# rrwick/Deepbinner

Hardware: AMD Instinct MI355X
Metric: reads classified/sec (1024-sample windows, batch 256) (higher is better)
Workload: dtype f32

## Files before the change

deepbinner_amd/csrc/dbh_api.hip:

```cpp
#include <hip/hip_runtime.h>

#include <algorithm>
#include <cmath>
#include <cstdio>
#include <cstdlib>
#include <cstring>
#include <new>
#include <string>
#include <thread>
#include <utility>
#include <mutex>
#include <vector>

#include "../../include/deepbinner_hip.h"
#include "dbh_general.h"
#define DBH_FORWARD_NS dbh
#define DBH_TIMELINE 0
#include "dbh_forward.hip"
#undef DBH_FORWARD_NS
#undef DBH_TIMELINE
#define DBH_FORWARD_NS dbh_timeline
#define DBH_TIMELINE 1
#include "dbh_forward.hip"
#undef DBH_FORWARD_NS
#undef DBH_TIMELINE

namespace {

thread_local std::string g_last_error;

int hip_fail(hipError_t e, const char* what) {
    g_last_error = std::string(what) + ": " + hipGetErrorString(e);
    return e == hipErrorOutOfMemory ? DBH_ERR_OUT_OF_MEMORY : DBH_ERR_HIP;
}

#define DBH_HIP(call)                                         \
    do {                                                      \
        hipError_t e_ = (call);                               \
        if (e_ != hipSuccess) return hip_fail(e_, #call);     \
    } while (0)

struct CanonConv { int k, cin, cout; };
void canon_convs(int n_classes, CanonConv out[dbh::kNumConvs]) {
    for (int i = 0; i < dbh::kNumConvs; ++i) {
        out[i].k = dbh::kConv[i].taps;
        out[i].cin = dbh::kConv[i].cin;
        out[i].cout = (i == dbh::kNumConvs - 1) ? n_classes : dbh::kConv[i].cout_pad;
    }
}

int64_t canon_param_count(int n_classes) {
    CanonConv cc[dbh::kNumConvs];
    canon_convs(n_classes, cc);
    int64_t n = 0;
    for (int i = 0; i < dbh::kNumConvs; ++i) n += (int64_t)cc[i].k * cc[i].cin * cc[i].cout + cc[i].cout;
    for (int i = 0; i < dbh::kNumBn; ++i) n += 4 * dbh::kBnChannels[i];
    return n;
}

void pack_weights(const float* w, int n_classes, std::vector<float>& packed) {
    using namespace dbh;
    packed.assign(kPackedFloats, 0.f);
    CanonConv cc[kNumConvs];
    canon_convs(n_classes, cc);
    const float* bn_first = w;
    for (int i = 0; i < kNumConvs; ++i) bn_first += (size_t)cc[i].k * cc[i].cin * cc[i].cout + cc[i].cout;
    std::vector<double> fold_scale(48, 1.0), fold_shift(48, 0.0);
    {
        const float* q = bn_first + 4 * kBnChannels[0];
        const float *gamma = q, *beta = q + 48, *mean = q + 96, *var = q + 144;
        for (int c = 0; c < 48; ++c) {
            fold_scale[c] = (double)gamma[c] / std::sqrt((double)var[c] + 1e-3);
            fold_shift[c] = (double)beta[c] - (double)mean[c] * fold_scale[c];
        }
    }
    static_assert(kBnChannels[1] == 48 && kConv[4].cin == 48 && kConv[4].taps == 1, "");
    const float* p = w;
    for (int i = 0; i < kNumConvs; ++i) {
        const int k = cc[i].k, cin = cc[i].cin, cout = cc[i].cout;
        const float* kernel = p;
        const float* bias = p + (size_t)k * cin * cout;
        p = bias + cout;
        float* dst = packed.data() + weight_offset(i);
        if (i == 0) {
            for (int tap = 0; tap < 3; ++tap)
                for (int c = 0; c < cout; ++c) dst[tap * 48 + c] = kernel[(tap * cin) * cout + c];
        } else if (kConv[i].wino) {
            const int sp_n = cin / 8, nt = kConv[i].cout_pad / 16;
            const int n_xi = kConv[i].wino == 4 ? 6 : 4;
            static const double G23[4][3] = {{1, 0, 0}, {.5, .5, .5}, {.5, -.5, .5}, {0, 0, 1}};
            static const double G43[6][3] = {{1. / 4, 0, 0},
                                             {-1. / 6, -1. / 6, -1. / 6},
                                             {-1. / 6, 1. / 6, -1. / 6},
                                             {1. / 24, 1. / 12, 1. / 6},
                                             {1. / 24, -1. / 12, 1. / 6},
                                             {0, 0, 1}};
            for (int xi = 0; xi < n_xi; ++xi) {
                const double* G = kConv[i].wino == 4 ? G43[xi] : G23[xi];
                for (int sp = 0; sp < sp_n; ++sp)
                    for (int t = 0; t < nt; ++t)
                        for (int lane = 0; lane < 64; ++lane)
                            for (int e = 0; e < 2; ++e) {
                                const int ci = frag_cin(i, sp, lane >> 4, e);
                                const int co = 16 * t + (lane & 15);
                                double v = 0.0;
                                if (co < cout)
                                    for (int tap = 0; tap < 3; ++tap)
                                        v += G[tap] * (double)kernel[((size_t)tap * cin + ci) * cout + co];
                                const size_t idx =
                                    kConv[i].wino == 4
                                        ? (((((size_t)t * sp_n + sp) * 3 + (xi >> 1)) * 64 + lane) * 2 + (xi & 1)) * 2 + e
                                        : wino2_by_tile(i)
// ... 143 lines not shown

int launch_forward(dbh_model* m, const float* x_dev, int64_t n, float* probs_dev,
                   int debug_stage, float* debug_dev, hipStream_t stream,
                   const FusedInput& in = FusedInput()) {
    if (m->kind != DBH_MODEL_KIND_PERSISTENT) return DBH_ERR_UNSUPPORTED;
    if (n == 0) return DBH_OK;
    const int64_t kChunk = (int64_t)(1 << 20) * in.steps;
    for (int64_t off = 0; off < n; off += kChunk) {
        const int64_t cnt = (n - off < kChunk) ? (n - off) : kChunk;
        hipEvent_t ev_stop = nullptr;
        if (m->timing > 0 && (debug_stage < 0 || debug_stage >= 100)) {
            const int64_t pos = m->launch_counter++ % m->timing;
            if (pos == 0) {
                if (m->events_used == m->events.size()) {
                    hipEvent_t a, b;
                    DBH_HIP(hipEventCreate(&a));
                    DBH_HIP(hipEventCreate(&b));
                    m->events.emplace_back(a, b);
                }
                DBH_HIP(hipEventRecord(m->events[m->events_used].first, stream));
                m->open_stop = m->events[m->events_used].second;
                m->open_windows = 0;
            }
            if (m->open_stop && pos < m->timing_span) {
                m->open_windows += cnt;
                if (pos == m->timing_span - 1) {
                    ev_stop = m->open_stop;
                    m->open_stop = nullptr;
                }
            }
        }
        const bool one_per_group = debug_stage >= 0 && debug_stage != 301;
        const int64_t groups = (cnt + dbh::kGroup - 1) / dbh::kGroup;
        const unsigned grid = (unsigned)(one_per_group || groups < m->cus ? groups : m->cus);
        void** tail = in.tail;
        size_t* tail_bytes = in.tail_bytes;
        if (!tail) {
            size_t k = 0;
            while (k < m->tails.size() && m->tails[k].stream != stream) ++k;
            if (k == m->tails.size()) m->tails.push_back(dbh_model::Tail{stream, nullptr, 0});
            tail = &m->tails[k].ptr;
            tail_bytes = &m->tails[k].bytes;
        }
        {
            void* before = *tail;
            const int st = ensure(tail, tail_bytes, 256 + (size_t)grid * dbh::kWgScratchFloats * sizeof(float));
            if (st != DBH_OK) return st;
            if (*tail != before) DBH_HIP(hipMemsetAsync(*tail, 0, 256, stream));
        }
        dbh::ForwardArgs a;
        a.packed = m->d_packed;
        a.x = x_dev ? x_dev + off * dbh::kWindow : nullptr;
        a.probs = probs_dev ? probs_dev + off * m->n_classes : nullptr;
        a.debug_out = debug_dev ? debug_dev + off * dbh::kStageFloats[debug_stage < 0 || debug_stage > 7 ? 0 : debug_stage]
                                : nullptr;
        a.samples = in.samples;
        a.offsets = in.offsets ? (const long long*)(in.offsets + off / in.steps) : nullptr;
        a.calls = in.calls ? (int*)(in.calls + off / in.steps) : nullptr;
        a.tail_scratch = (float*)((char*)*tail + 256);
        a.win_counter = (debug_stage < 0 && m->windows_by_counter) ? (int*)*tail : nullptr;
        a.clock_out = nullptr;
        if (m->clock_probe && debug_stage < 0) {
            const int st = ensure(&m->d_clock, &m->clock_bytes,
                                  (size_t)grid * (4 + dbh::kPhaseMarks * dbh::kPhaseGroups) * sizeof(int64_t));
            if (st != DBH_OK) return st;
            a.clock_out = (long long*)m->d_clock;
            m->clock_grid = grid;
        }
        a.score_diff = in.score_diff;
        a.read0 = (long long)(in.read0 + off / in.steps);
        a.len_hint = (long long)in.len_hint;
        a.hint_cap = (long long)in.hint_cap;
        a.n_windows = (long long)cnt;
        a.n_classes = m->n_classes;
        a.debug_stage = debug_stage;
        a.steps = in.steps;
        a.side = in.side;
        a.phases = m->phase_probe ? 1 : 0;
        a.chunk4_min_left = m->chunk4_rounds * (int)grid;
        a.chunk2_min_left = m->chunk2_rounds * (int)grid;
        if (debug_stage == 300)
            hipLaunchKernelGGL(dbh_timeline::dbh_forward_kernel, dim3(grid), dim3(dbh::kThreads),
                               0, stream, reinterpret_cast<dbh_timeline::ForwardArgs&>(a));
        else
            hipLaunchKernelGGL(dbh::dbh_forward_kernel, dim3(grid), dim3(dbh::kThreads), 0, stream,
                               a);
        DBH_HIP(hipGetLastError());
        if (ev_stop) {
            DBH_HIP(hipEventRecord(ev_stop, stream));
            ++m->events_used;
            m->timed_windows += m->open_windows;
            m->timed_launches += m->timing_span;
        }
    }
    return DBH_OK;
}

inline int steps_for(int scan_size) { return scan_size / (dbh::kWindow / 2); }

inline int model_steps(const dbh_model* m, int scan_size) {
    const int half = m->input_size / 2;
    const int steps = scan_size / half;
    return (steps > 0 && steps * half == scan_size) ? steps : 0;
}

inline size_t align256(size_t bytes) { return (bytes + 255) & ~(size_t)255; }

size_t general_workspace(const dbh_model* m, int64_t n_reads, int steps) {
    const int64_t windows = n_reads * steps;
    return align256((size_t)windows * m->n_classes * sizeof(float)) +
           dbh_gen::activation_bytes(m->gen, windows);
}

int general_predict(dbh_model* m, const float* x_dev, int64_t n, float* probs_dev,
                    hipStream_t stream) {
    if (n == 0) return DBH_OK;
    size_t k = 0;
    while (k < m->gen_scratch.size() && m->gen_scratch[k].stream != stream) ++k;
    if (k == m->gen_scratch.size()) m->gen_scratch.push_back(dbh_model::Tail{stream, nullptr, 0});
    dbh_model::Tail& sc = m->gen_scratch[k];
    const int st = ensure(&sc.ptr, &sc.bytes, dbh_gen::activation_bytes(m->gen, n));
    if (st != DBH_OK) return st;
    DBH_HIP(dbh_gen::forward(m->gen, x_dev, nullptr, nullptr, 1, 0, n, probs_dev, sc.ptr, stream));
    return DBH_OK;
}

}

extern "C" {

const char* dbh_version(void) { return "deepbinner_hip 0.1 (gfx950)"; }

const char* dbh_status_string(int status) {
    switch (status) {
        case DBH_OK: return "ok";
        case DBH_ERR_INVALID_ARGUMENT: return "invalid argument";
        case DBH_ERR_NO_DEVICE: return "no HIP device available";
        case DBH_ERR_HIP: return "HIP runtime error";
        case DBH_ERR_BAD_WEIGHTS: return "weight blob does not match the Deepbinner architecture";
        case DBH_ERR_UNSUPPORTED: return "unsupported model geometry";
        case DBH_ERR_OUT_OF_MEMORY: return "out of device memory";
        case DBH_ERR_COMM: return "multi-device exchange failed";
        default: return "unknown status";
    }
}

const char* dbh_last_error(void) { return g_last_error.c_str(); }

int dbh_device_count(int* count) {
    if (!count) return DBH_ERR_INVALID_ARGUMENT;
    int n = 0;
    static const bool once = [] {
        const char* spin = std::getenv("DEEPBINNER_SPIN_WAIT");
        if (!(spin && spin[0] == '1')) {
            int devices = 0;
            if (hipGetDeviceCount(&devices) == hipSuccess)
                for (int d = 0; d < devices; ++d)
                    if (hipSetDevice(d) == hipSuccess)
                        (void)hipSetDeviceFlags(hipDeviceScheduleBlockingSync);
            if (devices > 0) (void)hipSetDevice(0);
            (void)hipGetLastError();
        }
        return true;
    }();
    (void)once;
    hipError_t e = hipGetDeviceCount(&n);
    if (e != hipSuccess) {
        *count = 0;
        hip_fail(e, "hipGetDeviceCount");
// ... 923 lines not shown
    int32_t* side_calls_host[2] = {start_calls_host, end_calls_host};
    for (int j = 0; j < 2; ++j)
        if (side_calls_host[j] && models[j])
            std::memcpy(side_calls_host[j],
                        h + in_small + ((const char*)d_side[j] - (const char*)d_status),
                        (size_t)n_reads * sizeof(int32_t));
    if (stream_status_host && n_streams) {
        const int32_t* sorted_status = (const int32_t*)(h + in_small);
        for (int64_t i = 0; i < n_streams; ++i)
            stream_status_host[order[(size_t)i]] = sorted_status[i];
    }
    if (stage_ms) {
        float ms = 0.f;
        for (int k = 0; k < 3; ++k) {
            stage_ms[k] = hipEventElapsedTime(&ms, ev[k], ev[k + 1]) == hipSuccess ? ms : -1.0;
        }
    }
    return done(DBH_OK);
}

void* dbh_host_alloc(size_t bytes, void* user) {
    (void)user;
    void* p = nullptr;
    if (hipHostMalloc(&p, bytes ? bytes : 1, hipHostMallocPortable) != hipSuccess) {
        (void)hipGetLastError();
        return nullptr;
    }
    return p;
}

void dbh_host_release(void* ptr, void* user) {
    (void)user;
    if (ptr) (void)hipHostFree(ptr);
}

int dbh_host_is_pinned(const void* ptr, size_t bytes, int* pinned) {
    if (!pinned) return DBH_ERR_INVALID_ARGUMENT;
    *pinned = is_pinned(ptr, bytes) ? 1 : 0;
    return DBH_OK;
}

int dbh_model_set_host_group(dbh_model* m, int64_t windows_per_group) {
    if (!m || windows_per_group < 0) return DBH_ERR_INVALID_ARGUMENT;
    if (m->kind != DBH_MODEL_KIND_PERSISTENT) return DBH_OK;
    m->host_group_windows = windows_per_group > 0 ? windows_per_group : dbh_model::kDefaultGroup;
    return DBH_OK;
}

int dbh_model_reserve_cus(dbh_model* m, int n_cus) {
    if (!m || n_cus < 0) return DBH_ERR_INVALID_ARGUMENT;
    if (m->kind != DBH_MODEL_KIND_PERSISTENT) return DBH_OK;
    m->cus = m->cus_total - n_cus > 1 ? m->cus_total - n_cus : 1;
    return DBH_OK;
}

int dbh_stage_floats(int stage, int64_t* floats_per_window) {
    if (!floats_per_window || stage < 0 || stage > 7) return DBH_ERR_INVALID_ARGUMENT;
    *floats_per_window = dbh::kStageFloats[stage];
    return DBH_OK;
}

int dbh_debug_forward(dbh_model* m, const float* x_host, int64_t n, int stage, float* out_host) {
    if (!m || n <= 0 || !x_host || !out_host || stage < 0 || stage > 7)
        return DBH_ERR_INVALID_ARGUMENT;
    if (m->kind != DBH_MODEL_KIND_PERSISTENT) return DBH_ERR_UNSUPPORTED;
    const size_t per = (size_t)dbh::kStageFloats[stage];
    int st = ensure(&m->d_in, &m->in_bytes, (size_t)n * dbh::kWindow * sizeof(float));
    if (st != DBH_OK) return st;
    st = ensure(&m->d_work, &m->work_bytes, (size_t)n * per * sizeof(float));
    if (st != DBH_OK) return st;
    DBH_HIP(hipMemcpyAsync(m->d_in, x_host, (size_t)n * dbh::kWindow * sizeof(float),
                           hipMemcpyHostToDevice, 0));
    DBH_HIP(hipMemsetAsync(m->d_work, 0, (size_t)n * per * sizeof(float), 0));
    st = launch_forward(m, (const float*)m->d_in, n, nullptr, stage, (float*)m->d_work, 0);
    if (st != DBH_OK) return st;
    DBH_HIP(hipMemcpyAsync(out_host, m->d_work, (size_t)n * per * sizeof(float),
                           hipMemcpyDeviceToHost, 0));
    DBH_HIP(hipStreamSynchronize(0));
    return DBH_OK;
}

int dbh_forward_kernel_info(int* threads_per_block, int* lds_bytes, int* vgprs) {
    hipFuncAttributes attr;
    DBH_HIP(hipFuncGetAttributes(&attr, (const void*)dbh::dbh_forward_kernel));
    if (threads_per_block) *threads_per_block = dbh::kThreads;
    if (lds_bytes) *lds_bytes = (int)attr.sharedSizeBytes;
    if (vgprs) *vgprs = attr.numRegs;
    return DBH_OK;
}

int dbh_forward_executed_mfmas(int n_classes, int64_t* mfmas_per_window,
                                int64_t* flop_per_window) {
    if (n_classes < 2 || n_classes > dbh::kMaxClasses) return DBH_ERR_INVALID_ARGUMENT;
    const int64_t n = dbh::forward_mfmas(n_classes);
    if (mfmas_per_window) *mfmas_per_window = n;
    if (flop_per_window) *flop_per_window = n * 2048;
    return DBH_OK;
}

int dbh_forward_truncated_dev(dbh_model* m, const float* x_dev, int64_t n, int last_stage,
                              dbh_stream stream) {
    if (!m || n <= 0 || !x_dev || last_stage < 0 || last_stage > 6) return DBH_ERR_INVALID_ARGUMENT;
    if (m->kind != DBH_MODEL_KIND_PERSISTENT) return DBH_ERR_UNSUPPORTED;
    return launch_forward(m, x_dev, n, nullptr, 100 + last_stage, nullptr, (hipStream_t)stream);
}

int dbh_forward_timeline(dbh_model* m, const float* x_host, int64_t n, int64_t* stamps_host) {
    if (!m || n <= 0 || !x_host || !stamps_host) return DBH_ERR_INVALID_ARGUMENT;
    if (m->kind != DBH_MODEL_KIND_PERSISTENT) return DBH_ERR_UNSUPPORTED;
    const size_t stamp_bytes = (size_t)n * dbh::kWaves * 64 * sizeof(int64_t);
    int st = ensure(&m->d_in, &m->in_bytes, (size_t)n * dbh::kWindow * sizeof(float));
    if (st != DBH_OK) return st;
    st = ensure(&m->d_work, &m->work_bytes, stamp_bytes);
    if (st != DBH_OK) return st;
    st = ensure(&m->d_out, &m->out_bytes, (size_t)n * m->n_classes * sizeof(float));
    if (st != DBH_OK) return st;
    DBH_HIP(hipMemcpyAsync(m->d_in, x_host, (size_t)n * dbh::kWindow * sizeof(float),
                           hipMemcpyHostToDevice, 0));
    DBH_HIP(hipMemsetAsync(m->d_work, 0, stamp_bytes, 0));
    {
        dbh_timeline::ForwardArgs a = {};
        a.packed = m->d_packed;
        a.x = (const float*)m->d_in;
        a.probs = (float*)m->d_out;
        a.debug_out = (float*)m->d_work;
        a.n_windows = (long long)n;
        a.n_classes = m->n_classes;
        a.debug_stage = 300;
        a.steps = 1;
        const unsigned grid = (unsigned)((n + dbh::kGroup - 1) / dbh::kGroup);
        st = ensure(&m->d_tail, &m->tail_bytes, (size_t)grid * dbh::kWgScratchFloats * sizeof(float));
        if (st != DBH_OK) return st;
        a.tail_scratch = (float*)m->d_tail;
        a.win_counter = nullptr;
        hipLaunchKernelGGL(dbh_timeline::dbh_forward_kernel, dim3(grid), dim3(dbh::kThreads), 0, 0, a);
    }
    DBH_HIP(hipGetLastError());
    DBH_HIP(hipMemcpyAsync(stamps_host, m->d_work, stamp_bytes, hipMemcpyDeviceToHost, 0));
    DBH_HIP(hipStreamSynchronize(0));
    return DBH_OK;
}

int dbh_forward_timeline_i16(dbh_model* m, const int16_t* samples_host, int64_t n,
                             int64_t* stamps_host) {
    if (!m || n <= 0 || !samples_host || !stamps_host) return DBH_ERR_INVALID_ARGUMENT;
    if (m->kind != DBH_MODEL_KIND_PERSISTENT) return DBH_ERR_UNSUPPORTED;
    const size_t stamp_bytes = (size_t)n * dbh::kWaves * 64 * sizeof(int64_t);
    const size_t sample_bytes = (size_t)n * dbh::kWindow * sizeof(int16_t);
    const size_t offset_bytes = (size_t)(n + 1) * sizeof(int64_t);
    int st = ensure(&m->d_in, &m->in_bytes, sample_bytes + offset_bytes + 16);
    if (st != DBH_OK) return st;
    st = ensure(&m->d_work, &m->work_bytes, stamp_bytes);
    if (st != DBH_OK) return st;
    st = ensure(&m->d_out, &m->out_bytes, (size_t)n * (m->n_classes + 1) * sizeof(float));
    if (st != DBH_OK) return st;
    std::vector<int64_t> offsets((size_t)n + 1);
    for (int64_t i = 0; i <= n; ++i) offsets[(size_t)i] = i * dbh::kWindow;
    char* d_offsets = (char*)m->d_in + ((sample_bytes + 7) & ~(size_t)7);
    DBH_HIP(hipMemcpyAsync(m->d_in, samples_host, sample_bytes, hipMemcpyHostToDevice, 0));
    DBH_HIP(hipMemcpyAsync(d_offsets, offsets.data(), offset_bytes, hipMemcpyHostToDevice, 0));
    DBH_HIP(hipMemsetAsync(m->d_work, 0, stamp_bytes, 0));
    DBH_HIP(hipStreamSynchronize(0));
    {
        dbh_timeline::ForwardArgs a = {};
        a.packed = m->d_packed;
        a.probs = (float*)m->d_out;
        a.debug_out = (float*)m->d_work;
// ... 140 lines not shown
```

deepbinner_amd/csrc/dbh_forward.hip:

```cpp
#include <hip/hip_runtime.h>
#include <type_traits>

#include "dbh_layout.h"

#ifndef DBH_EXP_A_DMA_UNDER_MFMA
#define DBH_EXP_A_DMA_UNDER_MFMA 1
#endif
#ifndef DBH_ABL
#define DBH_ABL 0
#endif

#ifndef DBH_FORWARD_NS
#define DBH_FORWARD_NS dbh
#endif
#ifndef DBH_TIMELINE
#define DBH_TIMELINE 0
#endif

#ifndef DBH_STATS0_IN_F
#define DBH_STATS0_IN_F 1
#endif
#ifndef DBH_Y_EARLY
#define DBH_Y_EARLY 1
#endif
#ifndef DBH_F_AHEAD_EARLY
#define DBH_F_AHEAD_EARLY 0
#endif
namespace DBH_FORWARD_NS {
using namespace dbh;

typedef float f4 __attribute__((ext_vector_type(4)));
typedef float f2 __attribute__((ext_vector_type(2)));

constexpr int kWaves = 8;
constexpr int kThreads = kWaves * 64;

__device__ __forceinline__ f4 mfma4(float a, float b, f4 c) {
    return __builtin_amdgcn_mfma_f32_16x16x4f32(a, b, c, 0, 0, 0);
}

__device__ __forceinline__ void mark_realtime(unsigned* ts, int id) {
#if DBH_TIMELINE
    if (ts) {
        const unsigned now = (unsigned)__builtin_amdgcn_s_memrealtime();
        asm volatile("v_writelane_b32 %0, %1, %2" : "+v"(*ts) : "s"(now), "n"(id));
    }
#else
    (void)ts;
    (void)id;
#endif
}
__device__ __forceinline__ void mark(unsigned* ts, int id) {
#if DBH_TIMELINE
    if (ts) {
        const unsigned now = (unsigned)__builtin_readcyclecounter();
        asm volatile("v_writelane_b32 %0, %1, %2" : "+v"(*ts) : "s"(now), "n"(id));
    }
#else
    (void)ts;
    (void)id;
#endif
}
__device__ __forceinline__ void flush_marks(unsigned* ts, long long* out, int lane) {
#if DBH_TIMELINE
    if (ts) {
        if (*ts != 0u) out[lane] = (long long)*ts;
        *ts = 0u;
    }
#else
    (void)ts;
    (void)out;
    (void)lane;
#endif
}

template <int CTRL>
__device__ __forceinline__ float dpp_move(float v) {
    return __builtin_bit_cast(
        float, __builtin_amdgcn_update_dpp(0, __builtin_bit_cast(int, v), CTRL, 0xF, 0xF, true));
}
__device__ __forceinline__ float row16_max(float v) {
    v = fmaxf(v, dpp_move<0xB1>(v));
    v = fmaxf(v, dpp_move<0x4E>(v));
    v = fmaxf(v, dpp_move<0x141>(v));
    return fmaxf(v, dpp_move<0x140>(v));
}
__device__ __forceinline__ float row16_sum(float v) {
    v += dpp_move<0xB1>(v);
    v += dpp_move<0x4E>(v);
    v += dpp_move<0x141>(v);
    return v + dpp_move<0x140>(v);
}
__device__ __forceinline__ float lane_value(float v, int src_lane) {
    return __builtin_bit_cast(float,
                              __builtin_amdgcn_readlane(__builtin_bit_cast(int, v), src_lane));
}

template <int I>
struct IntC {
    static constexpr int value = I;
};
struct NoSide {
    template <int I>
    __device__ __forceinline__ void operator()(IntC<I>) const {}
};
struct NoBegin {
    __device__ __forceinline__ void operator()() const {}
};
struct NoHook {
// ... 1894 lines not shown
                                                float* __restrict__ park, int tid, int lane,
                                                int wave, unsigned* ts, int ts_base,
                                                unsigned& pair_rounds, const Side& side,
                                                const After& after) {
    constexpr int TOWN = HIGH ? 2 : 0, SP0 = HIGH ? DBH_CONV7_LOW : 0;
    const int n = lane & 15, q = lane >> 4;
    const int m = wave & 3;
    EpiParams<3, true> ep;
    load_epi<CONV, BNI>(ep, lds, packed, n);
    const int pm_n = 2 * (n >> 2) + (n & 1) + 8 * ((n >> 1) & 1);
    const unsigned a_addr = lds_addr(lds + kActOff + (m * 64 + 4 * pm_n) * kS48 + 2 * q);
    const unsigned b_addr = lds_addr(lds + kSlot0 + lane * 4);
    const int park_off = (m >> 1) * 3072 + ((n >> 2) * 16 + (m & 1) * 8 + q) * 4 + (n & 3);
    typedef typename std::conditional<LAST, lds_float*, float*>::type ParkPtr;
    ParkPtr park_lane;
    if constexpr (LAST) park_lane = lds_pinned(lds + kPark7Lds + park_off);
    else park_lane = park + park_off;
    (void)tid;
    float* mine = lds + kX7 + wave * 512 + lane * 4;
    const float* theirs = lds + kX7 + (wave ^ 4) * 512 + lane * 4;
    W43U U;
    W43nsPipe pipe;
    f4 own[6], shared[6];
    w43ns_step<TOWN, SP0, !HIGH, 0>(U, a_addr, b_addr, pipe, own, shared, ep.b[TOWN], ep.b[1], side);
    mark(ts, ts_base);
    full_barrier();
    mark(ts, ts_base + 1);
    w43ns_step<TOWN, SP0, !HIGH, 6>(
        U, a_addr, b_addr, pipe, own, shared, ep.b[TOWN], ep.b[1], [&](auto tag) {
            constexpr int G = decltype(tag)::value;
            side(tag);
            if constexpr (G == 6) w43_epilogue_half_park<TOWN, ParkPtr>(own, 0, ep.sc[TOWN], ep.sh[TOWN], park_lane);
            if constexpr (G == 7) w43_epilogue_half_park<TOWN, ParkPtr>(own, 1, ep.sc[TOWN], ep.sh[TOWN], park_lane);
        });
    const bool in_flight = after();
    f2 y[2][4];
    w43_partial_outputs(shared, 0, y[0]);
    w43_partial_outputs(shared, 1, y[1]);
    constexpr int kKeep = HIGH ? 2 : 0, kShip = HIGH ? 0 : 2;
    *reinterpret_cast<f4*>(mine) = f4{y[0][kShip].x, y[0][kShip].y, y[1][kShip].x, y[1][kShip].y};
    *reinterpret_cast<f4*>(mine + 256) =
        f4{y[0][kShip + 1].x, y[0][kShip + 1].y, y[1][kShip + 1].x, y[1][kShip + 1].y};
    pair_signal(lds, 2 * m + (HIGH ? 1 : 0), lane);
    if constexpr (!LAST) mark(ts, ts_base + 2);
    pair_wait(lds, 2 * m + (HIGH ? 0 : 1), pair_rounds + 1);
    pair_rounds += 1;
    const f4 t0 = *reinterpret_cast<const f4*>(theirs);
    const f4 t1 = *reinterpret_cast<const f4*>(theirs + 256);
    const float sc = ep.sc[1], sh = ep.sh[1];
#pragma unroll
    for (int h = 0; h < 2; ++h)
#pragma unroll
        for (int e = 0; e < 2; ++e) {
            const float ya = y[h][kKeep][e] + t0[2 * h + e];
            const float yb = y[h][kKeep + 1][e] + t1[2 * h + e];
            float p = fmaxf(fmaxf(ya, yb), 0.f);
            p = fmaf(p, sc, sh);
            park_lane[(2 * e + (HIGH ? 1 : 0)) * 768 + 256 + h * 16] = p;
        }
    if constexpr (LAST) {
        (void)in_flight;
        lds_barrier();
    } else {
        lds_barrier();
    }
    mark(ts, LAST ? ts_base + 2 : ts_base + 3);
}

struct NoAfter {
    __device__ __forceinline__ bool operator()() const { return false; }
};
template <int CONV, int BNI, bool LAST, class Side, class After = NoAfter>
__device__ __forceinline__ void w43_nsplit_pooled_layer(float* lds, const float* __restrict__ packed,
                                                        float* __restrict__ park, int tid, int lane,
                                                        int wave, unsigned* ts, int ts_base,
                                                        unsigned& pair_rounds, const Side& side,
                                                        const After& after = After()) {
    static_assert(kConv[CONV].wino == 4 && kConv[CONV].cin == 48 && kConv[CONV].cout_pad == 48, "");
    if (wave < 4)
        w43_nsplit_half<CONV, BNI, false, LAST>(lds, packed, park, tid, lane, wave, ts, ts_base, pair_rounds, side, after);
    else
        w43_nsplit_half<CONV, BNI, true, LAST>(lds, packed, park, tid, lane, wave, ts, ts_base, pair_rounds, side, after);
}

template <int CONV, int KS, int NTW, bool BN>
struct SmallMRegs {
    static constexpr int TAPS = kConv[CONV].taps;
    static constexpr int SPTOT = kConv[CONV].cin / 8;
    static constexpr int SP = SPTOT / KS;
    static constexpr int NGROUPS = 3 / NTW;
    static constexpr int ACTIVE = KS * NGROUPS;
    static_assert(SP * KS == SPTOT && NGROUPS * NTW == 3 && ACTIVE <= kWaves, "bad split");
    f2 b[TAPS * SP * NTW];
    EpiParams<1, BN> ep;
    __device__ __forceinline__ void prefetch(const float* __restrict__ packed, int bn_index,
                                             int lane, int wave) {
        if (ACTIVE == kWaves || wave < ACTIVE) {
            const int t0 = (wave % NGROUPS) * NTW, ks = wave / NGROUPS;
            const float* b_lane = packed + weight_offset(CONV) + (ks * SP * 3 + t0) * 128 + lane * 2;
#pragma unroll
            for (int tap = 0; tap < TAPS; ++tap)
#pragma unroll
                for (int sp = 0; sp < SP; ++sp)
#pragma unroll
                    for (int t = 0; t < NTW; ++t)
                        b[(tap * SP + sp) * NTW + t] = *reinterpret_cast<const f2*>(
                            b_lane + ((tap * SPTOT + sp) * 3 + t) * 128);
        }
        prefetch_epilogue(packed, bn_index, lane, wave);
    }
    __device__ __forceinline__ void prefetch_epilogue(const float* __restrict__ packed,
                                                      int bn_index, int lane, int wave) {
        if (wave < 3) {
            const int ch = wave * 16 + (lane & 15);
            ep.load(packed + bias_offset(CONV) + ch,
                    packed + (BN ? bn_scale_offset(bn_index) : 0) + ch,
                    packed + (BN ? bn_shift_offset(bn_index) : 0) + ch);
        }
    }
    template <int K0, int K1>
    __device__ __forceinline__ void prefetch_slice(const float* __restrict__ packed, int lane,
                                                   int wave) {
        if (ACTIVE == kWaves || wave < ACTIVE) {
            const int t0 = (wave % NGROUPS) * NTW, ks = wave / NGROUPS;
            const __amdgpu_buffer_rsrc_t view = buffer_view(packed + weight_offset(CONV));
            const unsigned wave_bytes = (unsigned)((ks * SP * 3 + t0) * 128) * 4u;
            const unsigned lane_bytes = (unsigned)lane * 8u;
#pragma unroll
            for (int k = K0; k < K1; ++k) {
                const int t = k % NTW, sp = (k / NTW) % SP, tap = k / (NTW * SP);
                b[k] = buffer_load_f2(view, lane_bytes,
                                      wave_bytes + (unsigned)(((tap * SPTOT + sp) * 3 + t) * 128) * 4u);
            }
        }
    }
};

template <int CONV, int S_IN, int STRIDE, int KS, int NTW, bool POOL, bool BN, bool TO_GLOBAL = false,
          class PreBarrier = NoHook, class PostBarrier = NoHook, class Between = NoBetween>
__device__ __forceinline__ void small_m_layer(float* lds, const float* in_region, float* out_region,
                                              float* red, const SmallMRegs<CONV, KS, NTW, BN>& regs, int lane,
                                              int wave, unsigned* ts, int ts_base,
                                              const PreBarrier& pre_barrier = PreBarrier(),
                                              const PostBarrier& post_barrier = PostBarrier(),
                                              const Between& between = Between(),
                                              const EpiParams<1, BN>* ep_all = nullptr) {
    using R = SmallMRegs<CONV, KS, NTW, BN>;
    constexpr int TAPS = R::TAPS, SP = R::SP;
    const int n = lane & 15, q = lane >> 4;
    f4 acc[1][NTW];
    zero_acc(acc);
    if (wave < R::ACTIVE) {
        const int ks = wave / R::NGROUPS;
        const int first = (STRIDE == 2) ? 1 : 0;
        const float* a_lane = in_region + (first + n * STRIDE) * S_IN + 2 * q + ks * SP * 8;
        f4 odd[NTW];
#pragma unroll
        for (int t = 0; t < NTW; ++t) odd[t] = f4{0.f, 0.f, 0.f, 0.f};
#pragma unroll
        for (int tap = 0; tap < TAPS; ++tap) {
            f2 a[SP];
#pragma unroll
            for (int sp = 0; sp < SP; ++sp)
                a[sp] = *reinterpret_cast<const f2*>(a_lane + tap * S_IN + sp * 8);
#pragma unroll
            for (int sp = 0; sp < SP; ++sp)
// ... 562 lines not shown
                    cnt = first_cnt;
                    pad = first_pad;
                    thirds_mode = thirds_ahead ? 0 : 2;
                } else {
                    thirds_mode = 1;
                    const float* st = lds + kStageStats + k * 8;
                    mean = reinterpret_cast<const double*>(st)[0];
                    inv = reinterpret_cast<const double*>(st)[1];
                    cnt = reinterpret_cast<const int*>(st)[4];
                    pad = reinterpret_cast<const int*>(st)[5];
                }
                const short* smp = reinterpret_cast<const short*>(lds + kStage + k * kStageWin);
#pragma unroll
                for (int t = 0; t < 6; ++t) {
                    const int i = 8 * j - 2 + 2 * t + q - pad;
                    const bool inside = q < 3 && i >= 0 && i < cnt;
                    in_raw[t] = inside ? (int)smp[inside ? i : 0] : kOutside;
                }
            }
            inv *= (double)kActScale;
#pragma unroll
            for (int t = 0; t < 6; ++t)
                in_a.xs[t] = in_raw[t] != kOutside ? (float)(((double)in_raw[t] - mean) * inv) : 0.f;
            mark(ts, 54);
        }
        if (win_counter != nullptr && tid == 0 && k == 0) taken = atomicAdd(win_counter, chunk_next);
        if (weights_cold) full_barrier();
#pragma unroll
        for (int g = 0; g < 3; ++g) in_a.w[g] = bw_a[g];
        in_a.p4_edge = j == 0 ? f2{0.f, 0.f} : f2{4.f, 4.f};
        in_a.one_edge = j == 127 ? f2{0.f, 0.f} : f2{1.f, 1.f};
        in_a.dump_on = debug_stage == 0;
        in_a.dump = nullptr;
        if (in_a.dump_on)
            in_a.dump = glob(args()->debug_out) + (long)win * kStageFloats[0] + 4 * j * 48 + 4 * q;
        in_a.stop = stop_stage == 0;
        in_a.wave_hi = wave >= 4;
        in_a.dump_b = debug_stage == 1;
        mark(ts, 1);
    }

    phase_add(9, ac_since);
    stage_b_chain(
        lds, packed, tid, lane, wave, ts, chain_windows, in_a, thirds_mode != 0,
        [&](int i) {
            if (thirds_mode == 2 && i < (2 * kWinoHalf / 256 + kWaves - 1) / kWaves)
                dma_weights_one<2 * kWinoHalf>(packed + weight_offset(1) + kWinoHalf, lds + kSlot1,
                                               lane, wave, i);
            if (thirds_mode == 1 && i < (kWinoHalf / 256 + kWaves - 1) / kWaves)
                dma_weights_one<kWinoHalf>(packed + weight_offset(1) + kWinoHalf, lds + kSlot1, lane,
                                           wave, i);
        },
        [&] {
            if (win_counter != nullptr && tid == 0 && k == 0)
                reinterpret_cast<int*>(lds + kNextWin)[0] = taken;
        },
        [&] { return glob(args()->debug_out) + (long)win * kStageFloats[1]; },
        lds + ((k > 0 && !weights_cold) ? kChainP : kSlot0));
    if (stop_stage == 0 || stop_stage == 1) {
        full_barrier();
        if (tid < kSyncWords) reinterpret_cast<unsigned*>(lds + kSync)[tid] = 0u;
        chain_windows = 0;
        full_barrier();
        continue;
    }
    if (k == 0 && win_counter != nullptr) {
        next_start = kGroup * (int)gridDim.x + reinterpret_cast<const int*>(lds + kNextWin)[0];
        const int left = n_windows - next_start;
        next_n = left <= 0 ? 0 : left < chunk_next ? left : chunk_next;
    }

    phase_add(10, ac_since);
    if (k == group_n - 1) {
        flush_marks(ts, ts_out, lane);
        break;
    }
    {
        auto third_step = [&](const float* src, float* dst, int step) {
            constexpr int NW = DBH_DMA_WAVES;
            constexpr int per_wave = (kWinoHalf / 256 + NW - 1) / NW;
            if (2 * step < per_wave) dma_weights_one<kWinoHalf, NW>(src, dst, lane, wave, 2 * step);
            if (2 * step + 1 < per_wave) dma_weights_one<kWinoHalf, NW>(src, dst, lane, wave, 2 * step + 1);
        };
        w43_nsplit_pooled_layer<6, 2, false>(
            lds, packed, wg_scratch + kWgPark7Off + k * kPark7Floats, tid, lane, wave, ts, 22, pair_rounds,
            [&](auto tag) {
                constexpr int G = decltype(tag)::value;
                if constexpr (G < 3) third_step(packed + weight_offset(1), lds + kChainP, G);
                if constexpr (G >= 6) third_step(packed + weight_offset(1) + 2 * kWinoHalf, lds + kSlot2, G - 6);
            });
    }
    phase_add(11, ac_since);
    if (stop_stage == 2) {
        full_barrier();
        if (debug_stage < 100) {
            float* out = glob(args()->debug_out) + (long)win * kStageFloats[2];
            const float* pk = wg_scratch + kWgPark7Off + k * kPark7Floats;
            for (int idx = tid; idx < 128 * 48; idx += kThreads) {
                const int p = idx / 48, c = idx - p * 48;
                const int hf = p >> 6, nn = (p >> 2) & 15, i = p & 3, g = c >> 4, qq = (c >> 2) & 3, r = c & 3;
                out[idx] = pk[hf * 3072 + (i * 3 + g) * 256 + (qq * 16 + nn) * 4 + r] * kActUnscale;
            }
        }
        continue;
    }
    flush_marks(ts, ts_out, lane);
    }

    if (stop_stage != 0 && stop_stage != 1) {
    int tid = tid_entry;
    asm volatile("" : "+v"(tid));
    const __attribute__((address_space(1))) float* packed_opaque =
        (const __attribute__((address_space(1))) float*)packed_entry;
    __attribute__((address_space(1))) float* scratch_opaque =
        (__attribute__((address_space(1))) float*)wg_scratch_entry;
    asm volatile("" : "+s"(packed_opaque), "+s"(scratch_opaque));
    const float* __restrict__ packed = (const float*)packed_opaque;
    float* const wg_scratch = (float*)scratch_opaque;
    const int lane = tid & 63;
    const int wave = __builtin_amdgcn_readfirstlane(tid >> 6);
    unsigned ts_acc = 0u;
    unsigned* ts = nullptr;
    long long* ts_out = nullptr;
    if (debug_stage >= 300) {
        ts = &ts_acc;
        ts_out = reinterpret_cast<long long*>(glob(args()->debug_out)) +
                 ((long)(group_start + (wave >> 1 < group_n ? wave >> 1 : 0)) * kWaves + wave) * 64;
    }
    const bool seam_b2 = samples_entry != nullptr;

    const int k_last = group_n - 1;
    const bool own_last = (wave >> 1) == k_last;
    f2 Y[3][2][4];
    unsigned c7_since = phases_on ? (unsigned)__builtin_readcyclecounter() : 0u;
    {
        auto third_step = [&](const float* src, float* dst, int step) {
            constexpr int NW = DBH_DMA_WAVES;
            constexpr int per_wave = (kWinoHalf / 256 + NW - 1) / NW;
            if (2 * step < per_wave) dma_weights_one<kWinoHalf, NW>(src, dst, lane, wave, 2 * step);
            if (2 * step + 1 < per_wave) dma_weights_one<kWinoHalf, NW>(src, dst, lane, wave, 2 * step + 1);
        };
        w43_nsplit_pooled_layer<6, 2, true>(
            lds, packed, nullptr, tid, lane, wave, ts, 59, pair_rounds, [&](auto tag) {
                constexpr int G = decltype(tag)::value;
                if constexpr (G < 3) third_step(packed + weight_offset(7), lds + kDS0, G);
                else if constexpr (G < 6) third_step(packed + weight_offset(7) + kWinoHalf, lds + kDS1, G - 3);
#if DBH_Y_EARLY
                if constexpr (G == 6)
                    d_load_y(Y, (const float*)(wg_scratch + kWgPark7Off + (wave >> 1) * kPark7Floats +
                                               (wave & 1) * 3072 + lane * 4));
#endif
            },
            [&]() -> bool {
#if DBH_Y_EARLY
                return true;
#endif
                d_load_y(Y, (const float*)(wg_scratch + kWgPark7Off + (wave >> 1) * kPark7Floats +
                                           (wave & 1) * 3072 + lane * 4));
                return true;
            });
    }
    phase_add(12, c7_since);
    if (stop_stage == 2) {
        if (debug_stage < 100) {
            float* out = glob(args()->debug_out) + (long)(group_start + k_last) * kStageFloats[2];
            const float* pk = lds + kPark7Lds;
            for (int idx = tid; idx < 128 * 48; idx += kThreads) {
                const int p = idx / 48, c = idx - p * 48;
                const int hf = p >> 6, nn = (p >> 2) & 15, i = p & 3, g = c >> 4, qq = (c >> 2) & 3, r = c & 3;
                out[idx] = pk[hf * 3072 + (i * 3 + g) * 256 + (qq * 16 + nn) * 4 + r] * kActUnscale;
            }
        }
        full_barrier();
    } else {
    const long long* __restrict__ offsets_arg = glob(args()->offsets);
    const int steps_arg = args()->steps;
    const int side_arg = args()->side;
    if (own_last)
        d_load_y(Y, (const float*)(lds + kPark7Lds + (wave & 1) * 3072 + lane * 4));

    phase_add(13, c7_since);
    phase_stamp(1);
    f2 w17[27];
    long long noff0[kGroup], noff1[kGroup];
    int nstep[kGroup];
    EpiParams<1, true> ep17[2];
    auto fetch_f = [&]() {
#pragma unroll
        for (int r = 0; r < 2; ++r) {
            const int e = (r * kThreads + tid) % 192, ch = (e >> 6) * 16 + (e & 15);
            ep17[r].load(packed + bias_offset(16) + ch, packed + bn_scale_offset(5) + ch, packed + bn_shift_offset(5) + ch);
        }
        const __amdgpu_buffer_rsrc_t view = buffer_view(packed + weight_offset(16));
        const unsigned lane_bytes = (unsigned)lane * 8u;
#pragma unroll
        for (int tap = 0; tap < 3; ++tap)
#pragma unroll
            for (int sp = 0; sp < 3; ++sp)
#pragma unroll
                for (int t = 0; t < 3; ++t) {
                    const unsigned soff = (unsigned)(((tap * 24 + wave * 3 + sp) * 3 + t) * 128) * 4u;
                    asm volatile("buffer_load_dwordx2 %0, %1, %2, %3 offen"
                                 : "=v"(w17[(tap * 3 + sp) * 3 + t])
                                 : "v"(lane_bytes), "s"(view), "s"(soff)
                                 : "memory");
                }
#pragma unroll
        for (int w = 0; w < kGroup; ++w) {
            noff0[w] = 0;
            noff1[w] = 0;
            nstep[w] = 0;
            if (seam_b2 && w < next_n) {
                unsigned next_read;
                split_window((unsigned)(next_start + w), steps_arg, &next_read, &nstep[w]);
                unsigned lane_zero = 0;
                asm volatile("" : "+v"(lane_zero));
                noff0[w] = offsets_arg[next_read + lane_zero];
                noff1[w] = offsets_arg[next_read + lane_zero + 1];
            }
        }
    };
    {
        float* dump3 = nullptr;
        if (debug_stage == 3 && (wave >> 1) < group_n)
            dump3 = glob(args()->debug_out) + (long)(group_start + (wave >> 1)) * kStageFloats[3];
// ... 418 lines not shown
```

Before: 6.058 million.

## Add Winograd-point-split conv7 layer with paired-wave handoff as default kernel

Result: no change. 6.055 million (median of 2 runs) (-0.0%).

```diff
diff --git a/deepbinner_amd/csrc/dbh_api.hip b/deepbinner_amd/csrc/dbh_api.hip
--- a/deepbinner_amd/csrc/dbh_api.hip
+++ b/deepbinner_amd/csrc/dbh_api.hip
@@ -16,18 +16,37 @@
 #include "dbh_general.h"
 #define DBH_FORWARD_NS dbh
 #define DBH_TIMELINE 0
+#define DBH_HANDOFF 0
 #include "dbh_forward.hip"
 #undef DBH_FORWARD_NS
 #undef DBH_TIMELINE
-#define DBH_FORWARD_NS dbh_timeline
-#define DBH_TIMELINE 1
+#undef DBH_HANDOFF
+#define DBH_FORWARD_NS dbh_sched
+#define DBH_TIMELINE 0
+#define DBH_HANDOFF 1
 #include "dbh_forward.hip"
 #undef DBH_FORWARD_NS
 #undef DBH_TIMELINE
+#undef DBH_HANDOFF
+#define DBH_FORWARD_NS dbh_timeline
+#define DBH_TIMELINE 1
+#define DBH_HANDOFF 1
+#include "dbh_forward.hip"
+#undef DBH_FORWARD_NS
+#undef DBH_TIMELINE
+#undef DBH_HANDOFF
 
 namespace {
 
 thread_local std::string g_last_error;
+
+bool forward_pinned() {
+    static const bool pinned = [] {
+        const char* v = std::getenv("DEEPBINNER_FORWARD_SCHEDULE");
+        return v != nullptr && std::strcmp(v, "pinned") == 0;
+    }();
+    return pinned;
+}
 
 int hip_fail(hipError_t e, const char* what) {
     g_last_error = std::string(what) + ": " + hipGetErrorString(e);
@@ -337,9 +356,12 @@
         if (debug_stage == 300)
             hipLaunchKernelGGL(dbh_timeline::dbh_forward_kernel, dim3(grid), dim3(dbh::kThreads),
                                0, stream, reinterpret_cast<dbh_timeline::ForwardArgs&>(a));
-        else
+        else if (forward_pinned())
             hipLaunchKernelGGL(dbh::dbh_forward_kernel, dim3(grid), dim3(dbh::kThreads), 0, stream,
                                a);
+        else
+            hipLaunchKernelGGL(dbh_sched::dbh_forward_kernel, dim3(grid), dim3(dbh::kThreads), 0,
+                               stream, reinterpret_cast<dbh_sched::ForwardArgs&>(a));
         DBH_HIP(hipGetLastError());
         if (ev_stop) {
             DBH_HIP(hipEventRecord(ev_stop, stream));
@@ -1429,7 +1451,8 @@
 
 int dbh_forward_kernel_info(int* threads_per_block, int* lds_bytes, int* vgprs) {
     hipFuncAttributes attr;
-    DBH_HIP(hipFuncGetAttributes(&attr, (const void*)dbh::dbh_forward_kernel));
+    DBH_HIP(hipFuncGetAttributes(&attr, forward_pinned() ? (const void*)dbh::dbh_forward_kernel
+                                                         : (const void*)dbh_sched::dbh_forward_kernel));
     if (threads_per_block) *threads_per_block = dbh::kThreads;
     if (lds_bytes) *lds_bytes = (int)attr.sharedSizeBytes;
     if (vgprs) *vgprs = attr.numRegs;
diff --git a/deepbinner_amd/csrc/dbh_forward.hip b/deepbinner_amd/csrc/dbh_forward.hip
--- a/deepbinner_amd/csrc/dbh_forward.hip
+++ b/deepbinner_amd/csrc/dbh_forward.hip
@@ -25,6 +25,15 @@
 #endif
 #ifndef DBH_F_AHEAD_EARLY
 #define DBH_F_AHEAD_EARLY 0
+#endif
+#ifndef DBH_HANDOFF
+#define DBH_HANDOFF 0
+#endif
+#undef DBH_CONV7_LAYER
+#if DBH_HANDOFF
+#define DBH_CONV7_LAYER w43_psplit_pooled_layer
+#else
+#define DBH_CONV7_LAYER w43_nsplit_pooled_layer
 #endif
 namespace DBH_FORWARD_NS {
 using namespace dbh;
@@ -2085,6 +2094,226 @@
     else
         w43_nsplit_half<CONV, BNI, true, LAST>(lds, packed, park, tid, lane, wave, ts, ts_base, pair_rounds, side, after);
 }
+
+#if DBH_HANDOFF
+struct W43pU {
+    f2 u[3][6];
+};
+struct W43psPipe {
+    f2 rows[2][5];
+    f4 b4[2];
+    f2 b2[2];
+};
+
+template <bool HIGH, int SP>
+__device__ __forceinline__ void w43p_transform(W43pU& U, const f2 (&d)[5]) {
+    const f2 m4 = f2{-4.f, -4.f}, p2 = f2{2.f, 2.f}, m2 = f2{-2.f, -2.f};
+    const f2 p4 = f2{4.f, 4.f}, m5 = f2{-5.f, -5.f};
+    if constexpr (!HIGH) {
+        const f2 a = __builtin_elementwise_fma(m4, d[2], d[4]), b = __builtin_elementwise_fma(m4, d[1], d[3]);
+        U.u[0][SP] = __builtin_elementwise_fma(p4, d[0], __builtin_elementwise_fma(m5, d[2], d[4]));
+        U.u[1][SP] = a + b;
+        U.u[2][SP] = a - b;
+    } else {
+        const f2 c = d[3] - d[1], g = d[2] - d[0];
+        U.u[0][SP] = __builtin_elementwise_fma(p2, g, c);
+        U.u[1][SP] = __builtin_elementwise_fma(m2, g, c);
+        U.u[2][SP] = __builtin_elementwise_fma(p4, d[0], __builtin_elementwise_fma(m5, d[2], d[4]));
+    }
+#pragma unroll
+    for (int x = 0; x < 3; ++x) asm volatile("" : "+v"(U.u[x][SP]));
+}
+
+template <int G>
+constexpr int w43ps_tile() { return G < 6 ? 2 : G < 12 ? 0 : 1; }
+
+template <bool HIGH, int G, class Side>
+__device__ __forceinline__ void w43ps_step(W43pU& U, unsigned a_addr, unsigned b_addr, W43psPipe& pipe,
+                                           f4 (&acc)[3], float bias, const Side& side) {
+    constexpr int R0 = HIGH ? 1 : 0;
+    auto loads = [&](auto step_tag) {
+        constexpr int N = decltype(step_tag)::value;
+        constexpr int T = w43ps_tile<N>(), SP = N % 6;
+        if constexpr (N < 6) {
+            pipe.rows[N & 1][0] = ds_read_f2<((R0 + 0) * kS48 + SP * 8) * 4>(a_addr);
+            pipe.rows[N & 1][1] = ds_read_f2<((R0 + 1) * kS48 + SP * 8) * 4>(a_addr);
+            pipe.rows[N & 1][2] = ds_read_f2<((R0 + 2) * kS48 + SP * 8) * 4>(a_addr);
+            pipe.rows[N & 1][3] = ds_read_f2<((R0 + 3) * kS48 + SP * 8) * 4>(a_addr);
+            pipe.rows[N & 1][4] = ds_read_f2<((R0 + 4) * kS48 + SP * 8) * 4>(a_addr);
+        }
+        pipe.b4[N & 1] = ds_read_f4<(T * kWinoHalf + (SP * 3 + (HIGH ? 2 : 0)) * 256) * 4>(b_addr);
+        pipe.b2[N & 1] = ds_read_f2<(T * kWinoHalf + (SP * 3 + 1) * 256) * 4 + (HIGH ? 8 : 0)>(b_addr);
+    };
+    constexpr int SP = G % 6;
+    if constexpr (G == 0) loads(IntC<0>{});
+    if constexpr (G + 1 < 18) {
+        loads(IntC<G + 1>{});
+        if constexpr (G + 1 < 6) asm volatile("s_waitcnt lgkmcnt(7)" ::: "memory");
+        else asm volatile("s_waitcnt lgkmcnt(2)" ::: "memory");
+    } else {
+        asm volatile("s_waitcnt lgkmcnt(0)" ::: "memory");
+    }
+    f4& b4 = pipe.b4[G & 1];
+    f2& b2 = pipe.b2[G & 1];
+    asm volatile("" : "+v"(b4));
+    asm volatile("" : "+v"(b2));
+    progress_priority<SP, 6>();
+    if constexpr (G < 6) {
+        f2(&d)[5] = pipe.rows[G & 1];
+#pragma unroll
+        for (int k = 0; k < 5; ++k) asm volatile("" : "+v"(d[k]));
+        __builtin_amdgcn_sched_barrier(0);
+        w43p_transform<HIGH, SP>(U, d);
+    }
+    __builtin_amdgcn_sched_barrier(0);
+    constexpr int X2 = HIGH ? 0 : 2, X4 = HIGH ? 1 : 0;
+    if constexpr (SP == 0) {
+        const f4 zero = f4{0.f, 0.f, 0.f, 0.f};
+        acc[X4] = mfma4(U.u[X4][SP].x, b4[0], zero);
+        acc[X4 + 1] = mfma4(U.u[X4 + 1][SP].x, b4[2], HIGH ? zero : f4{bias, bias, bias, bias});
+        acc[X2] = mfma4(U.u[X2][SP].x, b2[0], zero);
+    } else {
+        acc[X4] = mfma4(U.u[X4][SP].x, b4[0], acc[X4]);
+        acc[X4 + 1] = mfma4(U.u[X4 + 1][SP].x, b4[2], acc[X4 + 1]);
+        acc[X2] = mfma4(U.u[X2][SP].x, b2[0], acc[X2]);
+    }
+    acc[X4] = mfma4(U.u[X4][SP].y, b4[1], acc[X4]);
+    acc[X4 + 1] = mfma4(U.u[X4 + 1][SP].y, b4[3], acc[X4 + 1]);
+    acc[X2] = mfma4(U.u[X2][SP].y, b2[1], acc[X2]);
+#pragma unroll
+    for (int x = 0; x < 3; ++x) asm volatile("" : "+v"(acc[x]));
+    __builtin_amdgcn_sched_barrier(0);
+    side(IntC<G>{});
+    __builtin_amdgcn_sched_barrier(0);
+    if constexpr (SP != 5)
+        w43ps_step<HIGH, G + 1>(U, a_addr, b_addr, pipe, acc, bias, side);
+}
+
+template <bool HIGH>
+__device__ __forceinline__ void w43p_partial_outputs(const f4 (&acc)[3], int h, f2 (&y)[4]) {
+    const f2 a0 = f2{acc[0][2 * h], acc[0][2 * h + 1]}, a1 = f2{acc[1][2 * h], acc[1][2 * h + 1]};
+    const f2 a2 = f2{acc[2][2 * h], acc[2][2 * h + 1]};
+    if constexpr (!HIGH) {
+        const f2 s12 = a1 + a2, d12 = a1 - a2;
+        y[0] = a0 + s12;
+        y[1] = d12;
+        y[2] = s12;
+        y[3] = d12;
+    } else {
+        const f2 s34 = a0 + a1, d34 = a0 - a1;
+        y[0] = s34;
+        y[1] = d34 * f2{2.f, 2.f};
+        y[2] = s34 * f2{4.f, 4.f};
+        y[3] = __builtin_elementwise_fma(f2{8.f, 8.f}, d34, a2);
+    }
+}
+
+template <bool HIGH>
+__device__ __forceinline__ void w43p_ship(const f2 (&y)[2][4], float* mine) {
+    constexpr int kShip = HIGH ? 0 : 2;
+    *reinterpret_cast<f4*>(mine) = f4{y[0][kShip].x, y[0][kShip].y, y[1][kShip].x, y[1][kShip].y};
+    *reinterpret_cast<f4*>(mine + 256) =
+        f4{y[0][kShip + 1].x, y[0][kShip + 1].y, y[1][kShip + 1].x, y[1][kShip + 1].y};
+}
+
+template <bool HIGH, int T, class Ptr>
+__device__ __forceinline__ void w43p_finish(const f2 (&y)[2][4], f4 t0, f4 t1, float sc, float sh,
+                                            Ptr park_lane) {
+    constexpr int kKeep = HIGH ? 2 : 0;
+#pragma unroll
+    for (int h = 0; h < 2; ++h)
+#pragma unroll
+        for (int e = 0; e < 2; ++e) {
+            const float ya = y[h][kKeep][e] + t0[2 * h + e];
+            const float yb = y[h][kKeep + 1][e] + t1[2 * h + e];
+            float p = fmaxf(fmaxf(ya, yb), 0.f);
+            p = fmaf(p, sc, sh);
+            park_lane[(2 * e + (HIGH ? 1 : 0)) * 768 + T * 256 + h * 16] = p;
+        }
+}
+
+template <int CONV, int BNI, bool HIGH, bool LAST, class Side, class After>
+__device__ __forceinline__ void w43_psplit_half(float* lds, const float* __restrict__ packed,
+                                                float* __restrict__ park, int tid, int lane,
+                                                int wave, unsigned* ts, int ts_base,
+                                                unsigned& pair_rounds, const Side& side,
+                                                const After& after) {
+    const int n = lane & 15, q = lane >> 4;
+    const int m = wave & 3;
+    EpiParams<3, true> ep;
+    load_epi<CONV, BNI>(ep, lds, packed, n);
+    const int pm_n = 2 * (n >> 2) + (n & 1) + 8 * ((n >> 1) & 1);
+    const unsigned a_addr = lds_addr(lds + kActOff + (m * 64 + 4 * pm_n) * kS48 + 2 * q);
+    const unsigned b_addr = lds_addr(lds + kSlot0 + lane * 4);
+    const int park_off = (m >> 1) * 3072 + ((n >> 2) * 16 + (m & 1) * 8 + q) * 4 + (n & 3);
+    typedef typename std::conditional<LAST, lds_float*, float*>::type ParkPtr;
+    ParkPtr park_lane;
+    if constexpr (LAST) park_lane = lds_pinned(lds + kPark7Lds + park_off);
+    else park_lane = park + park_off;
+    (void)tid;
+    constexpr int kXB = LAST ? kSlot2 : kActOff;
+    float* mine_a = lds + kX7 + wave * 512 + lane * 4;
+    const float* theirs_a = lds + kX7 + (wave ^ 4) * 512 + lane * 4;
+    float* mine_b = lds + kXB + wave * 512 + lane * 4;
+    const float* theirs_b = lds + kXB + (wave ^ 4) * 512 + lane * 4;
+    const int word_mine = 2 * m + (HIGH ? 1 : 0), word_theirs = 2 * m + (HIGH ? 0 : 1);
+    W43pU U;
+    W43psPipe pipe;
+    f4 acc[3];
+    f2 y2[2][4], y0[2][4], y1[2][4];
+    w43ps_step<HIGH, 0>(U, a_addr, b_addr, pipe, acc, ep.b[2], side);
+    mark(ts, ts_base);
+    full_barrier();
+    mark(ts, ts_base + 1);
+    w43p_partial_outputs<HIGH>(acc, 0, y2[0]);
+    w43p_partial_outputs<HIGH>(acc, 1, y2[1]);
+    w43p_ship<HIGH>(y2, mine_a);
+    pair_signal(lds, word_mine, lane);
+    w43ps_step<HIGH, 6>(U, a_addr, b_addr, pipe, acc, ep.b[0], side);
+    w43p_partial_outputs<HIGH>(acc, 0, y0[0]);
+    w43p_partial_outputs<HIGH>(acc, 1, y0[1]);
+    pair_wait(lds, word_theirs, pair_rounds + 1);
+    const f4 t20 = *reinterpret_cast<const f4*>(theirs_a);
+    const f4 t21 = *reinterpret_cast<const f4*>(theirs_a + 256);
+    w43p_ship<HIGH>(y0, mine_b);
+    pair_signal(lds, word_mine, lane);
+    w43p_finish<HIGH, 2, ParkPtr>(y2, t20, t21, ep.sc[2], ep.sh[2], park_lane);
+    w43ps_step<HIGH, 12>(U, a_addr, b_addr, pipe, acc, ep.b[1], side);
+    const bool in_flight = after();
+    w43p_partial_outputs<HIGH>(acc, 0, y1[0]);
+    w43p_partial_outputs<HIGH>(acc, 1, y1[1]);
+    pair_wait(lds, word_theirs, pair_rounds + 2);
+    const f4 t00 = *reinterpret_cast<const f4*>(theirs_b);
+    const f4 t01 = *reinterpret_cast<const f4*>(theirs_b + 256);
+    w43p_ship<HIGH>(y1, mine_a);
+    pair_signal(lds, word_mine, lane);
+    if constexpr (!LAST) mark(ts, ts_base + 2);
+    w43p_finish<HIGH, 0, ParkPtr>(y0, t00, t01, ep.sc[0], ep.sh[0], park_lane);
+    pair_wait(lds, word_theirs, pair_rounds + 3);
+    pair_rounds += 3;
+    const f4 t10 = *reinterpret_cast<const f4*>(theirs_a);
+    const f4 t11 = *reinterpret_cast<const f4*>(theirs_a + 256);
+    w43p_finish<HIGH, 1, ParkPtr>(y1, t10, t11, ep.sc[1], ep.sh[1], park_lane);
+    (void)in_flight;
+    lds_barrier();
+    mark(ts, LAST ? ts_base + 2 : ts_base + 3);
+}
+static_assert((kSlot2 * 4) % 16 == 0 && kSlot2 + 8 * 512 <= kSlot2 + kWinoHalf, "");
+static_assert(kActOff + 8 * 512 <= kX7, "exchange buffer B below exchange buffer A");
+
+template <int CONV, int BNI, bool LAST, class Side, class After = NoAfter>
+__device__ __forceinline__ void w43_psplit_pooled_layer(float* lds, const float* __restrict__ packed,
+                                                        float* __restrict__ park, int tid, int lane,
+                                                        int wave, unsigned* ts, int ts_base,
+                                                        unsigned& pair_rounds, const Side& side,
+                                                        const After& after = After()) {
+    static_assert(kConv[CONV].wino == 4 && kConv[CONV].cin == 48 && kConv[CONV].cout_pad == 48, "");
+    if (wave < 4)
+        w43_psplit_half<CONV, BNI, false, LAST>(lds, packed, park, tid, lane, wave, ts, ts_base, pair_rounds, side, after);
+    else
+        w43_psplit_half<CONV, BNI, true, LAST>(lds, packed, park, tid, lane, wave, ts, ts_base, pair_rounds, side, after);
+}
+#endif
 
 template <int CONV, int KS, int NTW, bool BN>
 struct SmallMRegs {
@@ -2813,7 +3042,7 @@
             if (2 * step < per_wave) dma_weights_one<kWinoHalf, NW>(src, dst, lane, wave, 2 * step);
             if (2 * step + 1 < per_wave) dma_weights_one<kWinoHalf, NW>(src, dst, lane, wave, 2 * step + 1);
         };
-        w43_nsplit_pooled_layer<6, 2, false>(
+        DBH_CONV7_LAYER<6, 2, false>(
             lds, packed, wg_scratch + kWgPark7Off + k * kPark7Floats, tid, lane, wave, ts, 22, pair_rounds,
             [&](auto tag) {
                 constexpr int G = decltype(tag)::value;
@@ -2871,7 +3100,7 @@
             if (2 * step < per_wave) dma_weights_one<kWinoHalf, NW>(src, dst, lane, wave, 2 * step);
             if (2 * step + 1 < per_wave) dma_weights_one<kWinoHalf, NW>(src, dst, lane, wave, 2 * step + 1);
         };
-        w43_nsplit_pooled_layer<6, 2, true>(
+        DBH_CONV7_LAYER<6, 2, true>(
             lds, packed, nullptr, tid, lane, wave, ts, 59, pair_rounds, [&](auto tag) {
                 constexpr int G = decltype(tag)::value;
                 if constexpr (G < 3) third_step(packed + weight_offset(7), lds + kDS0, G);
```
